# yanyan-li/PlanarSLAM

Hardware: AMD Instinct MI355X
Metric: RGB-D frames/sec (extract+match+pose-opt) @640x480; 1->8-GPU batch scaling (higher is better)
Workload: dtype u8/f64

## Files before the change

### planarslam_amd/csrc/lsd.hip

```cpp
#include "common.h"
#include "ref_arith.h"
#include "wave_ops.h"
#include "lsd_nfa.h"
#include "isort.h"

namespace planar {
namespace lsd {

constexpr double LSD_PI = 3.14159265358979323846;
constexpr double M_3_2_PI = 3 * LSD_PI / 2, M_2__PI = 2 * LSD_PI;
constexpr float NOTDEF_F = -1024.0f;
constexpr double DEG_TO_RADS = LSD_PI / 180;
constexpr double RELATIVE_ERROR_FACTOR = 100.0;
constexpr int N_BINS = 1024;
constexpr int MAX_SEGS = 2048;
constexpr int MAX_RECTS = 4096;
constexpr int RING = 512;
constexpr int USED_LDS_BITS = 32768;

struct Plan {
    int W, H, w, h;
    int taps7[7], taps5[5];
    double rho, prec, p, log_nt, density_th, log_eps;
    int min_reg_size;
// ... 1126 lines not shown
    while (hole > top && sort_comp(s.key[first + parent], vk)) {
        s.key[first + hole] = s.key[first + parent]; s.idx[first + hole] = s.idx[first + parent];
        hole = parent;
        parent = (hole - 1) / 2;
    }
    s.key[first + hole] = vk; s.idx[first + hole] = vi;
}
__device__ void heap_sort_range(const SortBuf& s, int first, int last) {
    const int len = last - first;
    if (len >= 2) {
        int parent = (len - 2) / 2;
        while (true) {
            adjust_heap(s, first, parent, len, s.key[first + parent], s.idx[first + parent]);
            if (parent == 0) break;
            parent--;
        }
    }
    int l = last;
    while (l - first > 1) {
        --l;
        const float vk = s.key[l]; const int vi = s.idx[l];
        s.key[l] = s.key[first]; s.idx[l] = s.idx[first];
        adjust_heap(s, first, 0, l - first, vk, vi);
    }
}
__device__ void std_sort_desc(const SortBuf& s, int n) {
    if (n <= 0) return;
    int stack_first[64], stack_last[64], stack_depth[64], sp = 0;
    int lg = 0; { int t = n; while (t > 1) { t >>= 1; lg++; } }
    stack_first[sp] = 0; stack_last[sp] = n; stack_depth[sp] = 2 * lg; sp++;
    while (sp > 0) {
        sp--;
        int first = stack_first[sp], last = stack_last[sp], depth = stack_depth[sp];
        while (last - first > 16) {
            if (depth == 0) { heap_sort_range(s, first, last); break; }
            --depth;
            const int mid = first + (last - first) / 2;
            const int a = first + 1, bb = mid, c = last - 1;
            if (sort_comp(s.key[a], s.key[bb])) {
                if (sort_comp(s.key[bb], s.key[c])) sort_swap(s, first, bb);
                else if (sort_comp(s.key[a], s.key[c])) sort_swap(s, first, c);
                else sort_swap(s, first, a);
            } else if (sort_comp(s.key[a], s.key[c])) sort_swap(s, first, a);
            else if (sort_comp(s.key[bb], s.key[c])) sort_swap(s, first, c);
            else sort_swap(s, first, bb);
            int lo = first + 1, hi = last;
            const float pv = s.key[first];
            while (true) {
                while (sort_comp(s.key[lo], pv)) ++lo;
                --hi;
                while (sort_comp(pv, s.key[hi])) --hi;
                if (!(lo < hi)) break;
                sort_swap(s, lo, hi);
                ++lo;
            }
            const int cut = lo;
            stack_first[sp] = cut; stack_last[sp] = last; stack_depth[sp] = depth; sp++;
            last = cut;
        }
    }
    auto linear_insert = [&](int last) {
        const float vk = s.key[last]; const int vi = s.idx[last];
        int next = last - 1;
        while (sort_comp(vk, s.key[next])) { s.key[last] = s.key[next]; s.idx[last] = s.idx[next]; last = next; --next; }
        s.key[last] = vk; s.idx[last] = vi;
    };
    auto insertion = [&](int first, int last) {
        for (int i = first + 1; i < last; ++i) {
            if (sort_comp(s.key[i], s.key[first])) {
                const float vk = s.key[i]; const int vi = s.idx[i];
                for (int j = i; j > first; --j) { s.key[j] = s.key[j - 1]; s.idx[j] = s.idx[j - 1]; }
                s.key[first] = vk; s.idx[first] = vi;
            } else linear_insert(i);
        }
    };
    if (n > 16) { insertion(0, 16); for (int i = 16; i < n; ++i) linear_insert(i); }
    else insertion(0, n);
}

__device__ inline planar_keyline make_keyline(const Seg& sg, int cols, int rows, int class_id) {
    float e[4] = {sg.x1, sg.y1, sg.x2, sg.y2};
    if (e[0] < 0) e[0] = 0;
    if (e[0] >= cols) e[0] = (float)cols - 1.0f;
    if (e[2] < 0) e[2] = 0;
    if (e[2] >= cols) e[2] = (float)cols - 1.0f;
    if (e[1] < 0) e[1] = 0;
    if (e[1] >= rows) e[1] = (float)rows - 1.0f;
    if (e[3] < 0) e[3] = 0;
    if (e[3] >= rows) e[3] = (float)rows - 1.0f;
    planar_keyline kl;
    const float octaveScale = 1.0f;
    kl.start_x = e[0] * octaveScale; kl.start_y = e[1] * octaveScale; kl.end_x = e[2] * octaveScale; kl.end_y = e[3] * octaveScale;
    kl.s_oct_x = e[0]; kl.s_oct_y = e[1]; kl.e_oct_x = e[2]; kl.e_oct_y = e[3];
    const double d0 = (double)(e[0] - e[2]), d1 = (double)(e[1] - e[3]);
    kl.line_length = (float)sqrt(d0 * d0 + d1 * d1);
    const int ax = (int)rintf(e[0]), ay = (int)rintf(e[1]), bx = (int)rintf(e[2]), by = (int)rintf(e[3]);
    kl.num_pixels = max(abs(bx - ax), abs(by - ay)) + 1;
    kl.angle = (float)atan2((double)(kl.end_y - kl.start_y), (double)(kl.end_x - kl.start_x));
    kl.class_id = class_id;
    kl.octave = 0;
    kl.size = (kl.end_x - kl.start_x) * (kl.end_y - kl.start_y);
    kl.response = kl.line_length / (float)max(cols, rows);
    kl.pt_x = (kl.end_x + kl.start_x) / 2;
    kl.pt_y = (kl.end_y + kl.start_y) / 2;
    return kl;
}

__global__ __launch_bounds__(64) void lsd_keylines(const Plan* __restrict__ plan, uint8_t* __restrict__ ws, Misc* __restrict__ miscs, int max_lines,
                                                   planar_keyline* __restrict__ out_kl, double* __restrict__ out_eq, int32_t* __restrict__ n_out, int phase) {
    constexpr int LDS_SORT = 1024;
    __shared__ float key_l[LDS_SORT];
    __shared__ int idx_l[LDS_SORT];
    const Plan& P = *plan;
    const int b = blockIdx.x, lane = threadIdx.x;
    uint8_t* F = ws + (size_t)b * P.frame_bytes;
    Misc* misc = miscs + b;
    if (phase == 1 && !(misc->imp_done && misc->imp_redo && !misc->imp_full)) return;
    const bool partial = (phase == 0 || phase == 3) && misc->imp_done && !misc->imp_full;
    const Seg* segs = (const Seg*)(F + P.off_segs);
    const int n = min(misc->n_seg, MAX_SEGS);
    const int nk = min(n, max_lines);
    planar_keyline* K = out_kl + (size_t)b * max_lines;
    planar_keyline* Kws = (planar_keyline*)(F + P.off_kl);
    auto body = [&](float* key, int* idx) {
        for (int i = lane; i < n; i += 64) { key[i] = make_keyline(segs[i], P.W, P.H, i).response; idx[i] = i; }
        __threadfence_block();
        __syncthreads();
        if (n > max_lines) {
            if (lane == 0) { SortBuf s{key, idx}; std_sort_desc(s, n); }
            __threadfence_block();
            __syncthreads();
            if (partial) {
                bool tie = false;
                for (int i = lane; i < min(n - 1, max_lines); i += 64) tie = tie || key[i] == key[i + 1];
                if ((__ballot(tie) != 0ull || phase == 3) && lane == 0) misc->imp_redo = 1;
            }
        }
        for (int i = lane; i < nk; i += 64) {
            const planar_keyline kl = make_keyline(segs[idx[i]], P.W, P.H, n > max_lines ? i : idx[i]);
            K[i] = kl; Kws[i] = kl;
            const double sp0 = kl.start_x, sp1 = kl.start_y, ep0 = kl.end_x, ep1 = kl.end_y;
            const double l0 = sp1 * 1.0 - 1.0 * ep1, l1 = 1.0 * ep0 - sp0 * 1.0, l2 = sp0 * ep1 - sp1 * ep0;
            const double nrm = sqrt(l0 * l0 + l1 * l1 + l2 * l2);
            double* E = out_eq + ((size_t)b * max_lines + i) * 3;
            E[0] = l0 / nrm; E[1] = l1 / nrm; E[2] = l2 / nrm;
        }
    };
    if (n <= LDS_SORT) body(key_l, idx_l);
    else body((float*)(F + P.off_tmp), (int*)(F + P.off_tmp) + MAX_SEGS);
    if (lane == 0) { n_out[b] = misc->status ? 0 : nk; misc->n_kl = nk; }
}

constexpr int NUM_OF_BANDS = 9, WIDTH_OF_BAND = 7, LSP_H = 63;
__constant__ int LBD_COMB[32][2] = {{0, 1}, {0, 2}, {0, 3}, {0, 4}, {0, 5}, {0, 6}, {1, 2}, {1, 3}, {1, 4}, {1, 5}, {1, 6}, {2, 3}, {2, 4}, {2, 5}, {2, 6}, {2, 7},
                                    {2, 8}, {3, 4}, {3, 5}, {3, 6}, {3, 7}, {3, 8}, {4, 5}, {4, 6}, {4, 7}, {4, 8}, {5, 6}, {5, 7}, {5, 8}, {6, 7}, {6, 8}, {7, 8}};

__global__ __launch_bounds__(64) void lbd_describe(const Plan* __restrict__ plan, uint8_t* __restrict__ ws, const Misc* __restrict__ miscs, int max_lines,
                                                   uint8_t* __restrict__ out_desc, int B) {
    __shared__ float row[LSP_H][8];
    __shared__ float des[NUM_OF_BANDS * 8];
    const Plan& P = *plan;
    int b, li;
    xcd_frame_block(max_lines, B, b, li);
    const int lane = threadIdx.x;
    uint8_t* F = ws + (size_t)b * P.frame_bytes;
    const Misc* misc = miscs + b;
    if (li >= misc->n_kl) return;
    const planar_keyline L = ((const planar_keyline*)(F + P.off_kl))[li];
    const uint8_t* S5 = F + P.off_blur5;
    const short realWidth = (short)P.W, imageWidth = (short)(P.W - 1), imageHeight = (short)(P.H - 1);
    const short lengthOfLSP = (short)L.num_pixels;
    const short halfWidth = (lengthOfLSP - 1) / 2, halfHeight = (LSP_H - 1) / 2;
    const float lineMiddlePointX = (float)(0.5 * (L.s_oct_x + L.e_oct_x));
    const float lineMiddlePointY = (float)(0.5 * (L.s_oct_y + L.e_oct_y));
    float dL[2], dO[2];
    dL[0] = (float)cos((double)L.angle); dL[1] = (float)sin((double)L.angle);
    dO[0] = -dL[1]; dO[1] = dL[0];
    if (lane < LSP_H) {
        float sCorX0 = -dL[0] * halfWidth + dL[1] * halfHeight + lineMiddlePointX;
        float sCorY0 = -dL[1] * halfWidth - dL[0] * halfHeight + lineMiddlePointY;
        for (int h = 0; h < lane; h++) { sCorX0 -= dL[1]; sCorY0 += dL[0]; }
        float sCorX = sCorX0, sCorY = sCorY0;
        float pgdLRowSum = 0, ngdLRowSum = 0, pgdORowSum = 0, ngdORowSum = 0;
        for (short wID = 0; wID < lengthOfLSP; wID++) {
            short tempCor = (short)roundf(sCorX);
            const short xCor = (tempCor < 0) ? 0 : (tempCor > imageWidth) ? imageWidth : tempCor;
            tempCor = (short)roundf(sCorY);
            const short yCor = (tempCor < 0) ? 0 : (tempCor > imageHeight) ? imageHeight : tempCor;
            const uint8_t* r0 = S5 + (size_t)reflect101(yCor - 1, P.H) * realWidth;
            const uint8_t* r1 = S5 + (size_t)yCor * realWidth;
            const uint8_t* r2 = S5 + (size_t)reflect101(yCor + 1, P.H) * realWidth;
            const int xm = reflect101(xCor - 1, P.W), xp = reflect101(xCor + 1, P.W);
            const int a0 = r0[xm], a1 = r0[xCor], a2 = r0[xp], b0 = r1[xm], b2 = r1[xp], c0 = r2[xm], c1 = r2[xCor], c2 = r2[xp];
            const short dx = (short)((a2 - a0) + 2 * (b2 - b0) + (c2 - c0)), dy = (short)((c0 - a0) + 2 * (c1 - a1) + (c2 - a2));
            const float gDL = dx * dL[0] + dy * dL[1];
            const float gDO = dx * dO[0] + dy * dO[1];
            if (gDL > 0) pgdLRowSum += gDL; else ngdLRowSum -= gDL;
            if (gDO > 0) pgdORowSum += gDO; else ngdORowSum -= gDO;
            sCorX += dL[0];
            sCorY += dL[1];
        }
        const float coef = (float)P.gaussCoefG[lane];
        pgdLRowSum = coef * pgdLRowSum; ngdLRowSum = coef * ngdLRowSum;
        pgdORowSum = coef * pgdORowSum; ngdORowSum = coef * ngdORowSum;
        row[lane][0] = pgdLRowSum; row[lane][1] = ngdLRowSum; row[lane][2] = pgdLRowSum * pgdLRowSum; row[lane][3] = ngdLRowSum * ngdLRowSum;
        row[lane][4] = pgdORowSum; row[lane][5] = ngdORowSum; row[lane][6] = pgdORowSum * pgdORowSum; row[lane][7] = ngdORowSum * ngdORowSum;
    }
    __syncthreads();
    if (lane < NUM_OF_BANDS) {
        float sum[8] = {0, 0, 0, 0, 0, 0, 0, 0};
        const int h0 = max(0, (lane - 1) * WIDTH_OF_BAND), h1 = min(LSP_H, (lane + 2) * WIDTH_OF_BAND);
        for (int hID = h0; hID < h1; hID++) {
            const int own = hID / WIDTH_OF_BAND;
            float c;
            if (own == lane) c = (float)P.gaussCoefL[hID % WIDTH_OF_BAND + WIDTH_OF_BAND];
            else if (own == lane + 1) c = (float)P.gaussCoefL[hID % WIDTH_OF_BAND + 2 * WIDTH_OF_BAND];
            else c = (float)P.gaussCoefL[hID % WIDTH_OF_BAND];
            sum[0] += c * row[hID][0]; sum[1] += c * row[hID][1]; sum[2] += c * c * row[hID][2]; sum[3] += c * c * row[hID][3];
            sum[4] += c * row[hID][4]; sum[5] += c * row[hID][5]; sum[6] += c * c * row[hID][6]; sum[7] += c * c * row[hID][7];
        }
        const float invN2 = (float)(1.0 / (WIDTH_OF_BAND * 2.0)), invN3 = (float)(1.0 / (WIDTH_OF_BAND * 3.0));
        const float invN = (lane == 0 || lane == NUM_OF_BANDS - 1) ? invN2 : invN3;
        float* d = des + lane * 8;
        float temp = sum[0] * invN;
        d[0] = temp; d[4] = sqrtf(sum[2] * invN - temp * temp);
        temp = sum[1] * invN;
        d[1] = temp; d[5] = sqrtf(sum[3] * invN - temp * temp);
        temp = sum[4] * invN;
        d[2] = temp; d[6] = sqrtf(sum[6] * invN - temp * temp);
        temp = sum[5] * invN;
        d[3] = temp; d[7] = sqrtf(sum[7] * invN - temp * temp);
    }
    __syncthreads();
    if (lane == 0) {
        float tempM = 0, tempS = 0;
        for (int i = 0; i < NUM_OF_BANDS; i++) {
            const float* d = des + 8 * i;
            tempM += d[0] * d[0]; tempM += d[1] * d[1]; tempM += d[2] * d[2]; tempM += d[3] * d[3];
            tempS += d[4] * d[4]; tempS += d[5] * d[5]; tempS += d[6] * d[6]; tempS += d[7] * d[7];
        }
        tempM = 1 / sqrtf(tempM);
        tempS = 1 / sqrtf(tempS);
        for (int i = 0; i < NUM_OF_BANDS; i++) {
            float* d = des + 8 * i;
            d[0] *= tempM; d[1] *= tempM; d[2] *= tempM; d[3] *= tempM;
            d[4] *= tempS; d[5] *= tempS; d[6] *= tempS; d[7] *= tempS;
        }
        for (int i = 0; i < NUM_OF_BANDS * 8; i++) if ((double)des[i] > 0.4) des[i] = (float)0.4;
        float temp = 0;
        for (int i = 0; i < NUM_OF_BANDS * 8; i++) temp += des[i] * des[i];
        temp = 1 / sqrtf(temp);
        for (int i = 0; i < NUM_OF_BANDS * 8; i++) des[i] = des[i] * temp;
    }
    __syncthreads();
    if (lane < 32) {
        const float *f1 = &des[8 * LBD_COMB[lane][0]], *f2 = &des[8 * LBD_COMB[lane][1]];
        uint8_t result = 0;
        for (int i = 0; i < 8; i++) if (f1[i] > f2[i]) result += (uint8_t)(128 >> i);
        out_desc[((size_t)b * max_lines + li) * 32 + lane] = result;
    }
}

#ifdef PLANAR_TEST_HOOKS
__global__ __launch_bounds__(64) void debug_sort_kernel(float* key, int* idx, int n) {
    if (threadIdx.x == 0) { SortBuf s{key, idx}; std_sort_desc(s, n); }
}
#endif

}
}

using namespace planar;

struct planar_lsd {
    planar_ctx* ctx = nullptr;
    int W = 0, H = 0, max_batch = 0;
    lsd::Plan plan{};
    int detect_smem = 0;
    DevBuf d_plan, d_cx, d_cy, d_taps, d_ws, d_misc, d_lgamma;
    DevBuf d_in, d_kl, d_desc, d_eq, d_n;
    int stage_lines = 0;
    int pre_B = 0;
    int tie_order = 0;
    int top_only = 0;
    int sort_smem_g = 0, sort_smem_l = 0, sort_rows = 0, sort_rows_long = 0;
    LaunchProfile prof{4};
};

static void host_taps_q8(int ksize, double sigma, int* taps) {
    const double scale2X = -0.5 / (sigma * sigma);
    std::vector<double> v(ksize);
    double sum = 0;
    for (int i = 0; i < ksize; i++) { const double x = i - (ksize - 1) * 0.5; v[i] = std::exp(scale2X * x * x); sum += v[i]; }
    sum = 1. / sum;
    for (int i = 0; i < ksize; i++) taps[i] = (int)std::nearbyint(v[i] * sum * 256.0);
}
static bool host_exact_coefs(double inv_scale, int srcsize, int dstsize, std::vector<lsd::Coef>& out) {
    const double scale = 1.0 / inv_scale;
    out.assign(dstsize, lsd::Coef{0, 0, 0});
    if (srcsize < 2) return false;
    for (int val = 0; val < dstsize; val++) {
        const double fval = scale * ((double)val + 0.5) - 0.5;
        const int ival = (int)std::floor(fval);
        if (ival < 0) out[val] = lsd::Coef{0, 256, 0};
        else if (ival >= srcsize - 1) out[val] = lsd::Coef{srcsize - 2, 0, 256};
        else {
            out[val].ofs = ival;
            out[val].c1 = (int)std::nearbyint((fval - (double)ival) * 256.0);
            out[val].c0 = 256 - out[val].c1;
        }
    }
    return true;
}

extern "C" {

int planar_lsd_max_segments(void) { return lsd::MAX_SEGS; }

int planar_lsd_create(planar_ctx* ctx, int width, int height, int max_batch, planar_lsd** out) {
    PLANAR_REQUIRE(ctx && out, PLANAR_EINVAL, "null argument");
    *out = nullptr;
    PLANAR_REQUIRE(width >= 32 && height >= 32 && width <= 4096 && height <= 1280, PLANAR_EINVAL, "image size out of range (32..4096 x 32..1280)");
    PLANAR_REQUIRE(max_batch >= 1, PLANAR_EINVAL, "max_batch must be >= 1");
    PLANAR_HIP_CHECK(hipSetDevice(ctx->device));
    planar_lsd* o = new (std::nothrow) planar_lsd();
    PLANAR_REQUIRE(o != nullptr, PLANAR_ENOMEM, "host allocation failed");
    o->ctx = ctx; o->W = width; o->H = height; o->max_batch = max_batch;
    lsd::Plan& P = o->plan;
    const double SCALE = 0.8, SIGMA_SCALE = 0.6, QUANT = 2.0, ANG_TH = 22.5;
    P.W = width; P.H = height;
    P.w = (int)std::nearbyint(width * SCALE); P.h = (int)std::nearbyint(height * SCALE);
    P.prec = lsd::LSD_PI * ANG_TH / 180; P.p = ANG_TH / 180; P.rho = QUANT / std::sin(P.prec);
    P.density_th = 0.7; P.log_eps = 0;
    const double sigma = SIGMA_SCALE / SCALE;
    const unsigned hk = (unsigned)(std::ceil(sigma * std::sqrt(2 * 3.0 * std::log(10.0))));
    if (1 + 2 * (int)hk != 7) { delete o; set_error("planar_lsd_create: unexpected LSD Gaussian size"); return PLANAR_EINVAL; }
    host_taps_q8(7, sigma, P.taps7);
    host_taps_q8(5, 1.0, P.taps5);
    P.log_nt = 5 * (std::log10(double(P.w)) + std::log10(double(P.h))) / 2 + std::log10(11.0);
    P.min_reg_size = (int)(size_t)(-P.log_nt / std::log10(P.p));
    {
        double u = (7 * 3 - 1) / 2, sg = (7 * 2 + 1) / 2, inv = -1 / (2 * sg * sg);
        for (int i = 0; i < 21; i++) { const double dis = i - u; P.gaussCoefL[i] = std::exp(dis * dis * inv); }
        u = (9 * 7 - 1) / 2; sg = (9 * 7) / 2; inv = -1 / (2 * sg * sg);
        for (int i = 0; i < 63; i++) { const double dis = i - u; P.gaussCoefG[i] = std::exp(dis * dis * inv); }
    }
    std::vector<lsd::Coef> cx, cy;
    if (!host_exact_coefs(SCALE, width, P.w, cx) || !host_exact_coefs(SCALE, height, P.h, cy)) {
        delete o; set_error("planar_lsd_create: image too small to resample"); return PLANAR_EINVAL;
    }
    size_t off = 0;
    auto carve = [&](size_t bytes) { size_t o2 = off; off = align_up(off + bytes, (size_t)256); return o2; };
    const size_t NPf = (size_t)width * height, NPs = (size_t)P.w * P.h;
    P.off_blur7 = carve(NPf); P.off_blur5 = carve(NPf); P.off_dx = 0; P.off_dy = 0;
// ... 273 lines not shown
```

### planarslam_amd/csrc/orb.hip

```cpp
#include <algorithm>
#include <cmath>

#include "common.h"

namespace planar {
namespace orb {

constexpr int PATCH_SIZE = 31;
constexpr int HALF_PATCH = 15;
constexpr int EDGE_THRESHOLD = 19;
constexpr int MAX_LEVELS = 16;
constexpr int CELL_W = 30;
constexpr int RADIX_BITS = 4;

struct LevelDev {
    int w, h, pitch;
    int64_t off;
    int minBX, minBY, maxBX, maxBY;
    int nCols, nRows, wCell, hCell;
    int cell_begin, ncells;
    int cand_off, cand_cap;
    int nfeat;
    int depth;
    int nIni;
// ... 490 lines not shown
        c_n = 0;
        int it = head;
        while (it >= 0) {
            __threadfence_block();
            const int sz = n_hi[it] - n_lo[it];
            if (sz == 1) { it = n_next[it]; continue; }
            nToExpand += split(it);
            it = erase(it);
        }
        if (count >= N || count == prevSize) {
            finish = true;
        } else if (count + nToExpand * 3 > N) {
            while (!finish) {
                const int prevSize2 = count;
                { int* t; t = c_size; c_size = p_size; p_size = t; t = c_seq; c_seq = p_seq; p_seq = t; t = c_slot; c_slot = p_slot; p_slot = t; }
                p_n = c_n; c_n = 0;
                __threadfence_block();
                for (int step = 0; step < p_n; step++) {
                    unsigned long long best = 0;
                    for (int i = lane; i < p_n; i += 64) {
                        const int sz = p_size[i];
                        if (sz > 0) {
                            const unsigned long long v = ((unsigned long long)sz << 40) | ((unsigned long long)p_seq[i] << 16) | (unsigned)i;
                            best = v > best ? v : best;
                        }
                    }
#pragma unroll
                    for (int o = 32; o > 0; o >>= 1) { const unsigned long long t = __shfl_xor(best, o); best = t > best ? t : best; }
                    const int idx = (int)(best & 0xffffu);
                    const int slot = p_slot[idx];
                    if (lane == 0) p_size[idx] = 0;
                    __threadfence_block();
                    split(slot);
                    erase(slot);
                    if (count >= N) break;
                }
                if (count >= N || count == prevSize2) finish = true;
            }
        }
    }

    __threadfence_block();
    int pos = 0;
    const int cw = L.wCell, ch = L.hCell, ncols = L.nCols;
    for (int it = head; it >= 0; it = n_next[it], pos++) {
        const int lo = n_lo[it], hi = n_hi[it];
        unsigned long long best = 0;
        for (int i = lo + lane; i < hi; i += 64) {
            const uint32_t key = (uint32_t)S[i];
            const unsigned x = key & 0xfffu, y = (key >> 12) & 0xfffu, sc = key >> 24;
            const unsigned cell = ((y - 3) / ch) * ncols + (x - 3) / cw;
            const unsigned long long ord = ((unsigned long long)cell << 24) | (y << 12) | x;
            const unsigned long long v = ((unsigned long long)sc << 48) | ((~ord) & 0xffffffffffffull);
            best = v > best ? v : best;
        }
#pragma unroll
        for (int o = 32; o > 0; o >>= 1) { const unsigned long long t = __shfl_xor(best, o); best = t > best ? t : best; }
        if (lane == 0) {
            const unsigned long long ord = (~best) & 0xffffffffffffull;
            out[pos] = (uint32_t)(ord & 0xffffffu) | ((uint32_t)(best >> 48) << 24);
        }
    }
    if (lane == 0) *out_count = pos;
}

struct TileDev { short level, tx, ty, pad; };

__global__ __launch_bounds__(256) void orb_blur(const PlanDev* __restrict__ plan, const TileDev* __restrict__ tiles,
                                                const uint8_t* __restrict__ pyr, uint8_t* __restrict__ blur, int n_tiles, int B) {
    __shared__ uint32_t s_pw[22][19];
    __shared__ __attribute__((aligned(8))) uint16_t s_h[22][68];
    int frame, tile;
    xcd_frame_block(n_tiles, B, frame, tile);
    const TileDev T = tiles[tile];
    const LevelDev& L = plan->lv[T.level];
    const int tid = threadIdx.x;
    const int x0 = T.tx * 64, y0 = T.ty * 16;
    const uint8_t* img = pyr + (int64_t)frame * plan->pyr_stride + L.off;
    for (int i = tid; i < 22 * 18; i += 256) {
        const int r = i / 18, wq = i - r * 18;
        int y = y0 + r - 3;
        y = y < 0 ? -y : y; y = y >= L.h ? 2 * L.h - 2 - y : y; y = max(0, min(y, L.h - 1));
        const uint8_t* row = img + (int64_t)y * L.pitch;
        const int xs = x0 - 4 + 4 * wq;
        uint32_t w;
        if (xs >= 0 && xs + 3 < L.w) w = *(const uint32_t*)(row + xs);
        else {
            w = 0;
#pragma unroll
            for (int k = 0; k < 4; k++) {
                int x = xs + k;
                x = x < 0 ? -x : x; x = x >= L.w ? 2 * L.w - 2 - x : x; x = max(0, min(x, L.w - 1));
                w |= (uint32_t)row[x] << (8 * k);
            }
        }
        s_pw[r][wq] = w;
    }
    __syncthreads();
    for (int i = tid; i < 22 * 16; i += 256) {
        const int r = i >> 4, q = i & 15;
        const uint32_t w0 = s_pw[r][q], w1 = s_pw[r][q + 1], w2 = s_pw[r][q + 2];
        uint32_t b[10];
        b[0] = (w0 >> 8) & 255u; b[1] = (w0 >> 16) & 255u; b[2] = w0 >> 24;
        b[3] = w1 & 255u; b[4] = (w1 >> 8) & 255u; b[5] = (w1 >> 16) & 255u; b[6] = w1 >> 24;
        b[7] = w2 & 255u; b[8] = (w2 >> 8) & 255u; b[9] = (w2 >> 16) & 255u;
        uint32_t o[4];
#pragma unroll
        for (int j = 0; j < 4; j++) {
            const uint32_t v = 18u * (b[j] + b[j + 6]) + 34u * (b[j + 1] + b[j + 5]) + 49u * (b[j + 2] + b[j + 4]) + 55u * b[j + 3];
            o[j] = min(v, 65535u);
        }
        *(uint2*)&s_h[r][4 * q] = make_uint2(o[0] | (o[1] << 16), o[2] | (o[3] << 16));
    }
    __syncthreads();
    {
        const int c4 = (tid & 15) * 4, r = tid >> 4;
        uint32_t acc[4] = {0, 0, 0, 0};
        const uint32_t taps[7] = {18u, 34u, 49u, 55u, 49u, 34u, 18u};
#pragma unroll
        for (int k = 0; k < 7; k++) {
            const uint2 v = *(const uint2*)&s_h[r + k][c4];
            acc[0] += taps[k] * (v.x & 0xffffu); acc[1] += taps[k] * (v.x >> 16);
            acc[2] += taps[k] * (v.y & 0xffffu); acc[3] += taps[k] * (v.y >> 16);
        }
        uint32_t packed = 0;
#pragma unroll
        for (int i = 0; i < 4; i++) packed |= min((acc[i] + 32768u) >> 16, 255u) << (8 * i);
        const int y = y0 + r, x = x0 + c4;
        if (y < L.h && x < L.pitch)
            *(uint32_t*)(blur + (int64_t)frame * plan->pyr_stride + L.off + (int64_t)y * L.pitch + x) = packed;
    }
}

__device__ __forceinline__ float fast_atan2_deg(float y, float x) {
    const float scale = (float)(180 / 3.1415926535897932384626433832795);
    const float p1 = 0.9997878412794807f * scale, p3 = -0.3258083974640975f * scale;
    const float p5 = 0.1555786518463281f * scale, p7 = -0.04432655554792128f * scale;
    const float ax = fabsf(x), ay = fabsf(y);
    float a, c, c2;
    if (ax >= ay) {
        c = __fdiv_rn(ay, __fadd_rn(ax, 2.220446049250313e-16f));
        c2 = __fmul_rn(c, c);
        a = __fmul_rn(__fadd_rn(__fmul_rn(__fadd_rn(__fmul_rn(__fadd_rn(__fmul_rn(p7, c2), p5), c2), p3), c2), p1), c);
    } else {
        c = __fdiv_rn(ax, __fadd_rn(ay, 2.220446049250313e-16f));
        c2 = __fmul_rn(c, c);
        a = __fsub_rn(90.f, __fmul_rn(__fadd_rn(__fmul_rn(__fadd_rn(__fmul_rn(__fadd_rn(__fmul_rn(p7, c2), p5), c2), p3), c2), p1), c));
    }
    if (x < 0) a = __fsub_rn(180.f, a);
    if (y < 0) a = __fsub_rn(360.f, a);
    return a;
}

__global__ __launch_bounds__(256) void orb_describe(const PlanDev* __restrict__ plan, const uint8_t* __restrict__ pyr,
                                                    const uint8_t* __restrict__ blur, const uint32_t* __restrict__ kept,
                                                    const int* __restrict__ kept_count, planar_keypoint* __restrict__ kps,
                                                    uint8_t* __restrict__ desc, int32_t* __restrict__ n_out, int per_frame, int B) {
    int frame, bx;
    xcd_frame_block(per_frame, B, frame, bx);
    const int sub = threadIdx.x & 15;
    const int kpi = bx * 16 + (threadIdx.x >> 4);
    int level = -1, first = 0, total = 0;
    for (int l = 0; l < plan->nlevels; l++) {
        const int c = kept_count[frame * MAX_LEVELS + l];
        if (level < 0 && kpi < total + c) { level = l; first = total; }
        total += c;
    }
    if (bx == 0 && threadIdx.x == 0) n_out[frame] = total;
    if (level < 0) return;
    const LevelDev& L = plan->lv[level];
    const uint32_t key = kept[(int64_t)frame * plan->kept_stride + L.kept_off + (kpi - first)];
    const int x = (int)(key & 0xfffu) + L.minBX, y = (int)((key >> 12) & 0xfffu) + L.minBY;
    const int score = (int)(key >> 24);
    const int64_t lvl_off = (int64_t)frame * plan->pyr_stride + L.off;

    const uint8_t* c = pyr + lvl_off + (int64_t)y * L.pitch + x;
    int m10 = 0, m01 = 0;
    if (sub == 0) {
        for (int u = -HALF_PATCH; u <= HALF_PATCH; ++u) m10 += u * c[u];
    } else {
        const int d = plan->umax[sub];
        int vsum = 0;
        const uint8_t* cp = c + (int64_t)sub * L.pitch;
        const uint8_t* cm = c - (int64_t)sub * L.pitch;
        for (int u = -d; u <= d; ++u) {
            const int vp = cp[u], vm = cm[u];
            vsum += vp - vm;
            m10 += u * (vp + vm);
        }
        m01 = sub * vsum;
    }
#pragma unroll
    for (int o = 8; o > 0; o >>= 1) { m10 += __shfl_xor(m10, o); m01 += __shfl_xor(m01, o); }
    const float angle = fast_atan2_deg((float)m01, (float)m10);

    const float factorPI = (float)(3.1415926535897932384626433832795 / 180.f);
    const float ang = __fmul_rn(angle, factorPI);
    const float a = (float)cos((double)ang), b = (float)sin((double)ang);
    const uint8_t* bc = blur + lvl_off + (int64_t)y * L.pitch + x;
    const int step = L.pitch;
    uint32_t bits = 0;
    const signed char* pat = c_pattern + sub * 64;
#pragma unroll
    for (int i = 0; i < 16; i++) {
        const float x0 = (float)pat[4 * i], y0 = (float)pat[4 * i + 1], x1 = (float)pat[4 * i + 2], y1 = (float)pat[4 * i + 3];
        const int r0 = __float2int_rn(__fadd_rn(__fmul_rn(x0, b), __fmul_rn(y0, a)));
        const int q0 = __float2int_rn(__fsub_rn(__fmul_rn(x0, a), __fmul_rn(y0, b)));
        const int r1 = __float2int_rn(__fadd_rn(__fmul_rn(x1, b), __fmul_rn(y1, a)));
        const int q1 = __float2int_rn(__fsub_rn(__fmul_rn(x1, a), __fmul_rn(y1, b)));
        const int t0 = bc[r0 * step + q0], t1 = bc[r1 * step + q1];
        bits |= (uint32_t)(t0 < t1) << i;
    }
    const int64_t o = (int64_t)frame * plan->kp_cap + kpi;
    *(uint16_t*)(desc + o * 32 + sub * 2) = (uint16_t)bits;
    if (sub == 0) {
        planar_keypoint kp;
        kp.x = __fmul_rn((float)x, L.scale);
        kp.y = __fmul_rn((float)y, L.scale);
        kp.size = L.patch;
        kp.angle = angle;
        kp.response = (float)score;
        kp.octave = level;
        kp.class_id = -1;
        kps[o] = kp;
    }
}

}
}

using namespace planar;
using namespace planar::orb;

struct planar_orb {
    planar_ctx* ctx = nullptr;
    planar_orb_params params{};
    int W = 0, H = 0, max_batch = 0;
    PlanDev plan{};
    std::vector<CellDev> cells;
    std::vector<TileDev> tiles;
    std::vector<float> scale, inv_scale, sigma2, inv_sigma2;
    int fast_smem = 0, node_cap = 0, oct_smem = 0;
    int last_B = 0;
    DevBuf d_plan, d_cells, d_tiles, d_tabs, d_pyr, d_blur, d_cand, d_cell_count, d_sortA, d_sortB, d_level_count,
        d_kept, d_kept_count, d_dropped;
    DevBuf d_in, d_kps, d_desc, d_nout;
    std::vector<const char*> launch_names;
    LaunchProfile prof;
    explicit planar_orb(int nlevels) : prof(nlevels + 5) {}
};

static inline int cv_round_f(float v) { return (int)nearbyintf(v); }
static inline int cv_round_d(double v) { return (int)nearbyint(v); }
static inline short sat_short(float v) { int i = cv_round_f(v); return (short)std::min(32767, std::max(-32768, i)); }

extern "C" {

int planar_orb_create(planar_ctx* ctx, const planar_orb_params* p, int W, int H, int max_batch, planar_orb** out) {
    PLANAR_REQUIRE(ctx && p && out, PLANAR_EINVAL, "null argument");
    *out = nullptr;
    PLANAR_REQUIRE(p->nlevels >= 1 && p->nlevels <= MAX_LEVELS, PLANAR_EINVAL, "nlevels must be in [1,16]");
    PLANAR_REQUIRE(p->nfeatures >= 1 && p->nfeatures <= 60000, PLANAR_EINVAL, "nfeatures out of range");
    PLANAR_REQUIRE(p->scale_factor > 1.0f, PLANAR_EINVAL, "scale_factor must be > 1");
    PLANAR_REQUIRE(p->min_th_fast >= 1 && p->ini_th_fast >= p->min_th_fast && p->ini_th_fast <= 254, PLANAR_EINVAL,
                   "FAST thresholds must satisfy 1 <= min <= ini <= 254");
    PLANAR_REQUIRE(W >= 64 && H >= 64 && W <= 4096 && H <= 4096, PLANAR_EINVAL, "image size must be within [64,4096]");
    PLANAR_REQUIRE(max_batch >= 1, PLANAR_EINVAL, "max_batch must be >= 1");
    PLANAR_HIP_CHECK(hipSetDevice(ctx->device));

    planar_orb* o = new (std::nothrow) planar_orb(p->nlevels);
    PLANAR_REQUIRE(o != nullptr, PLANAR_ENOMEM, "host allocation failed");
    o->ctx = ctx; o->params = *p; o->W = W; o->H = H; o->max_batch = max_batch;
    const int nl = p->nlevels;
    const double scaleFactor = p->scale_factor;
    o->scale.resize(nl); o->sigma2.resize(nl); o->inv_scale.resize(nl); o->inv_sigma2.resize(nl);
    o->scale[0] = 1.0f; o->sigma2[0] = 1.0f;
    for (int i = 1; i < nl; i++) { o->scale[i] = (float)(o->scale[i - 1] * scaleFactor); o->sigma2[i] = o->scale[i] * o->scale[i]; }
    for (int i = 0; i < nl; i++) { o->inv_scale[i] = 1.0f / o->scale[i]; o->inv_sigma2[i] = 1.0f / o->sigma2[i]; }
    std::vector<int> nfeat(nl);
    {
        float factor = (float)(1.0f / scaleFactor);
        float nDesired = p->nfeatures * (1 - factor) / (1 - (float)std::pow((double)factor, (double)nl));
        int sum = 0;
        for (int l = 0; l < nl - 1; l++) { nfeat[l] = cv_round_f(nDesired); sum += nfeat[l]; nDesired *= factor; }
        nfeat[nl - 1] = std::max(p->nfeatures - sum, 0);
    }
    PlanDev& P = o->plan;
    memset(&P, 0, sizeof(P));
    {
        int v, v0, vmax = (int)std::floor(HALF_PATCH * std::sqrt(2.f) / 2 + 1);
        int vmin = (int)std::ceil(HALF_PATCH * std::sqrt(2.f) / 2);
        const double hp2 = HALF_PATCH * HALF_PATCH;
        for (v = 0; v <= vmax; ++v) P.umax[v] = cv_round_d(std::sqrt(hp2 - v * v));
        for (v = HALF_PATCH, v0 = 0; v >= vmin; --v) { while (P.umax[v0] == P.umax[v0 + 1]) ++v0; P.umax[v] = v0; ++v0; }
    }
    P.nlevels = nl; P.ini_th = p->ini_th_fast; P.min_th = p->min_th_fast;

    int64_t pyr_off = 0;
    int cand_off = 0, kept_off = 0, rs_off = 0;
    int max_tile_bytes = 0, max_nfeat = 0;
    std::vector<short4> tabs;
    for (int l = 0; l < nl; l++) {
        LevelDev& L = P.lv[l];
        L.w = cv_round_f((float)W * o->inv_scale[l]);
        L.h = cv_round_f((float)H * o->inv_scale[l]);
        L.minBX = L.minBY = EDGE_THRESHOLD - 3;
        L.maxBX = L.w - EDGE_THRESHOLD + 3; L.maxBY = L.h - EDGE_THRESHOLD + 3;
        const float width = (float)(L.maxBX - L.minBX), height = (float)(L.maxBY - L.minBY);
        L.nCols = (int)(width / CELL_W); L.nRows = (int)(height / CELL_W);
        if (L.nCols < 1 || L.nRows < 1 || L.w < 2 * EDGE_THRESHOLD + 8 || L.h < 2 * EDGE_THRESHOLD + 8) {
            delete o;
            set_error("planar_orb_create: pyramid level %d (%dx%d) is too small for the 30-px FAST cell grid", l, L.w, L.h);
            return PLANAR_EINVAL;
        }
        L.wCell = (int)std::ceil(width / L.nCols); L.hCell = (int)std::ceil(height / L.nRows);
        L.pitch = align_up(L.w, 16);
        L.off = pyr_off;
        pyr_off += align_up((int64_t)L.pitch * L.h, (int64_t)256);
        L.nfeat = nfeat[l];
        max_nfeat = std::max(max_nfeat, nfeat[l]);
        L.scale = o->scale[l];
        L.patch = (float)(int)(PATCH_SIZE * o->scale[l]);
        L.nIni = (int)std::round((float)(L.maxBX - L.minBX) / (L.maxBY - L.minBY));
        if (L.nIni < 1 || L.nIni > 64) {
            delete o;
            set_error("planar_orb_create: level %d aspect ratio gives %d initial octree nodes (supported: 1..64)", l, L.nIni);
            return PLANAR_EINVAL;
        }
        L.hX = (float)(L.maxBX - L.minBX) / L.nIni;
        int ext = std::max(L.maxBX - L.minBX, L.maxBY - L.minBY), D = 1;
        while ((1 << (D - 1)) < ext) D++;
        L.depth = D;
        int ini_bits = 0; while ((1 << ini_bits) < L.nIni) ini_bits++;
        L.code_bits = align_up(2 * D + ini_bits, RADIX_BITS);
        if (L.code_bits > 32) { delete o; set_error("planar_orb_create: path code needs %d bits", L.code_bits); return PLANAR_EINVAL; }
        L.cell_begin = (int)o->cells.size();
        L.cand_off = cand_off;
        for (int i = 0; i < L.nRows; i++) {
            const float iniY = (float)(L.minBY + i * L.hCell);
            float maxY = iniY + L.hCell + 6;
            if (iniY >= L.maxBY - 3) continue;
            if (maxY > L.maxBY) maxY = (float)L.maxBY;
            for (int j = 0; j < L.nCols; j++) {
                const float iniX = (float)(L.minBX + j * L.wCell);
                float maxX = iniX + L.wCell + 6;
                if (iniX >= L.maxBX - 6) continue;
                if (maxX > L.maxBX) maxX = (float)L.maxBX;
                CellDev C;
                C.level = (short)l;
                C.x0 = (short)((int)iniX + 3); C.y0 = (short)((int)iniY + 3);
                C.ww = (short)((int)maxX - 3 - C.x0); C.wh = (short)((int)maxY - 3 - C.y0);
                if (C.ww <= 0 || C.wh <= 0) continue;
                C.slot_off = cand_off;
// ... 250 lines not shown
```

Baseline: 12870.

## Stage LBD and ORB patch pixels in LDS tiles before gradient and BRIEF sampling

The LBD describer now processes each line in 64-pixel chunks. For each chunk it computes the bounding box of all 63 rows, loads that region of the blurred image into a shared-memory tile with coalesced 32-bit loads, and computes the Sobel gradients from LDS instead of scattered global byte reads. ORB describe likewise copies each keypoint's orientation disc and BRIEF sampling box into a per-keypoint LDS tile with word loads, then takes the moments and pattern comparisons from LDS. The aim is to replace many uncoalesced byte gathers from global memory, at the cost of extra LDS use that may lower occupancy, extra sync points, and box-size limits that rely on static_assert geometry.

```diff
diff --git a/planarslam_amd/csrc/lsd.hip b/planarslam_amd/csrc/lsd.hip
--- a/planarslam_amd/csrc/lsd.hip
+++ b/planarslam_amd/csrc/lsd.hip
@@ -1302,6 +1302,9 @@
 }
 
 constexpr int NUM_OF_BANDS = 9, WIDTH_OF_BAND = 7, LSP_H = 63;
+constexpr int LBD_CH = 64, LBD_BOX = 96, LBD_PITCH_DW = 25;
+static_assert(2 * (LBD_BOX - 6) * (LBD_BOX - 6) >= (LSP_H + LBD_CH) * (LSP_H + LBD_CH), "LBD_BOX >= ceil((63 + LBD_CH) / sqrt(2)) + 4, and two to spare");
+static_assert(LBD_PITCH_DW * 4 >= LBD_BOX + 3 && (LBD_PITCH_DW & 1) == 1, "a tile row holds the box and its misalignment; odd pitch in words");
 __constant__ int LBD_COMB[32][2] = {{0, 1}, {0, 2}, {0, 3}, {0, 4}, {0, 5}, {0, 6}, {1, 2}, {1, 3}, {1, 4}, {1, 5}, {1, 6}, {2, 3}, {2, 4}, {2, 5}, {2, 6}, {2, 7},
                                     {2, 8}, {3, 4}, {3, 5}, {3, 6}, {3, 7}, {3, 8}, {4, 5}, {4, 6}, {4, 7}, {4, 8}, {5, 6}, {5, 7}, {5, 8}, {6, 7}, {6, 8}, {7, 8}};
 
@@ -1309,6 +1312,7 @@
                                                    uint8_t* __restrict__ out_desc, int B) {
     __shared__ float row[LSP_H][8];
     __shared__ float des[NUM_OF_BANDS * 8];
+    __shared__ uint32_t tile[LBD_BOX * LBD_PITCH_DW];
     const Plan& P = *plan;
     int b, li;
     xcd_frame_block(max_lines, B, b, li);
@@ -1318,7 +1322,7 @@
     if (li >= misc->n_kl) return;
     const planar_keyline L = ((const planar_keyline*)(F + P.off_kl))[li];
     const uint8_t* S5 = F + P.off_blur5;
-    const short realWidth = (short)P.W, imageWidth = (short)(P.W - 1), imageHeight = (short)(P.H - 1);
+    const short imageWidth = (short)(P.W - 1), imageHeight = (short)(P.H - 1);
     const short lengthOfLSP = (short)L.num_pixels;
     const short halfWidth = (lengthOfLSP - 1) / 2, halfHeight = (LSP_H - 1) / 2;
     const float lineMiddlePointX = (float)(0.5 * (L.s_oct_x + L.e_oct_x));
@@ -1326,30 +1330,58 @@
     float dL[2], dO[2];
     dL[0] = (float)cos((double)L.angle); dL[1] = (float)sin((double)L.angle);
     dO[0] = -dL[1]; dO[1] = dL[0];
-    if (lane < LSP_H) {
-        float sCorX0 = -dL[0] * halfWidth + dL[1] * halfHeight + lineMiddlePointX;
-        float sCorY0 = -dL[1] * halfWidth - dL[0] * halfHeight + lineMiddlePointY;
-        for (int h = 0; h < lane; h++) { sCorX0 -= dL[1]; sCorY0 += dL[0]; }
-        float sCorX = sCorX0, sCorY = sCorY0;
-        float pgdLRowSum = 0, ngdLRowSum = 0, pgdORowSum = 0, ngdORowSum = 0;
-        for (short wID = 0; wID < lengthOfLSP; wID++) {
-            short tempCor = (short)roundf(sCorX);
-            const short xCor = (tempCor < 0) ? 0 : (tempCor > imageWidth) ? imageWidth : tempCor;
-            tempCor = (short)roundf(sCorY);
-            const short yCor = (tempCor < 0) ? 0 : (tempCor > imageHeight) ? imageHeight : tempCor;
-            const uint8_t* r0 = S5 + (size_t)reflect101(yCor - 1, P.H) * realWidth;
-            const uint8_t* r1 = S5 + (size_t)yCor * realWidth;
-            const uint8_t* r2 = S5 + (size_t)reflect101(yCor + 1, P.H) * realWidth;
-            const int xm = reflect101(xCor - 1, P.W), xp = reflect101(xCor + 1, P.W);
-            const int a0 = r0[xm], a1 = r0[xCor], a2 = r0[xp], b0 = r1[xm], b2 = r1[xp], c0 = r2[xm], c1 = r2[xCor], c2 = r2[xp];
-            const short dx = (short)((a2 - a0) + 2 * (b2 - b0) + (c2 - c0)), dy = (short)((c0 - a0) + 2 * (c1 - a1) + (c2 - a2));
-            const float gDL = dx * dL[0] + dy * dL[1];
-            const float gDO = dx * dO[0] + dy * dO[1];
-            if (gDL > 0) pgdLRowSum += gDL; else ngdLRowSum -= gDL;
-            if (gDO > 0) pgdORowSum += gDO; else ngdORowSum -= gDO;
-            sCorX += dL[0];
-            sCorY += dL[1];
-        }
+    const bool has_row = lane < LSP_H;
+    float sCorX = -dL[0] * halfWidth + dL[1] * halfHeight + lineMiddlePointX;
+    float sCorY = -dL[1] * halfWidth - dL[0] * halfHeight + lineMiddlePointY;
+    for (int h = 0; h < lane; h++) { sCorX -= dL[1]; sCorY += dL[0]; }
+    float pgdLRowSum = 0, ngdLRowSum = 0, pgdORowSum = 0, ngdORowSum = 0;
+    auto clampX = [&](float v) -> short { const short t = (short)roundf(v); return (t < 0) ? (short)0 : (t > imageWidth) ? imageWidth : t; };
+    auto clampY = [&](float v) -> short { const short t = (short)roundf(v); return (t < 0) ? (short)0 : (t > imageHeight) ? imageHeight : t; };
+    const int W = P.W, H = P.H, w3 = W & 3;
+    for (int w0 = 0; w0 < lengthOfLSP; w0 += LBD_CH) {
+        const int n = min(LBD_CH, (int)lengthOfLSP - w0);
+        float eX = sCorX, eY = sCorY;
+        for (int k = 1; k < n; k++) { eX += dL[0]; eY += dL[1]; }
+        const int xs = clampX(sCorX), ys = clampY(sCorY), xe = clampX(eX), ye = clampY(eY);
+        const int xs0 = __builtin_amdgcn_readlane(xs, 0), xs1 = __builtin_amdgcn_readlane(xs, LSP_H - 1), xe0 = __builtin_amdgcn_readlane(xe, 0), xe1 = __builtin_amdgcn_readlane(xe, LSP_H - 1);
+        const int ys0 = __builtin_amdgcn_readlane(ys, 0), ys1 = __builtin_amdgcn_readlane(ys, LSP_H - 1), ye0 = __builtin_amdgcn_readlane(ye, 0), ye1 = __builtin_amdgcn_readlane(ye, LSP_H - 1);
+        const int x_lo = max(min(min(xs0, xs1), min(xe0, xe1)) - 1, 0), x_hi = min(max(max(xs0, xs1), max(xe0, xe1)) + 1, W - 1);
+        const int y_lo = max(min(min(ys0, ys1), min(ye0, ye1)) - 1, 0), y_hi = min(max(max(ys0, ys1), max(ye0, ye1)) + 1, H - 1);
+        const int bw = x_hi - x_lo + 1, bh = min(y_hi - y_lo + 1, LBD_BOX);
+        const int m0 = (int)(((uintptr_t)S5 + (size_t)y_lo * W + x_lo) & 3);
+        lds_sync();
+        const int nw = bh * LBD_PITCH_DW;
+        for (int i0 = lane; i0 < nw; i0 += 64 * 8) {
+            uint32_t v[8];
+#pragma unroll
+            for (int u = 0; u < 8; u++) {
+                const int i = min(i0 + 64 * u, nw - 1), r = i / LBD_PITCH_DW, q = i - r * LBD_PITCH_DW;
+                const int mis = (m0 + r * w3) & 3;
+                v[u] = *(const uint32_t*)(S5 + (size_t)(y_lo + r) * W + (x_lo - mis + (4 * q < mis + bw ? 4 * q : 0)));
+            }
+#pragma unroll
+            for (int u = 0; u < 8; u++) tile[min(i0 + 64 * u, nw - 1)] = v[u];
+        }
+        lds_sync();
+        if (has_row) {
+            const uint8_t* T = (const uint8_t*)tile;
+            auto row_at = [&](int y) { const int r = y - y_lo; return r * (LBD_PITCH_DW * 4) + ((m0 + r * w3) & 3) - x_lo; };
+            for (int k = 0; k < n; k++) {
+                const short xCor = clampX(sCorX), yCor = clampY(sCorY);
+                const int r0 = row_at(yCor == 0 ? 1 : yCor - 1), r1 = row_at(yCor), r2 = row_at(yCor == imageHeight ? H - 2 : yCor + 1);
+                const int xm = xCor == 0 ? 1 : xCor - 1, xp = xCor == imageWidth ? W - 2 : xCor + 1;
+                const int a0 = T[r0 + xm], a1 = T[r0 + xCor], a2 = T[r0 + xp], b0 = T[r1 + xm], b2 = T[r1 + xp], c0 = T[r2 + xm], c1 = T[r2 + xCor], c2 = T[r2 + xp];
+                const short dx = (short)((a2 - a0) + 2 * (b2 - b0) + (c2 - c0)), dy = (short)((c0 - a0) + 2 * (c1 - a1) + (c2 - a2));
+                const float gDL = dx * dL[0] + dy * dL[1];
+                const float gDO = dx * dO[0] + dy * dO[1];
+                if (gDL > 0) pgdLRowSum += gDL; else ngdLRowSum -= gDL;
+                if (gDO > 0) pgdORowSum += gDO; else ngdORowSum -= gDO;
+                sCorX += dL[0];
+                sCorY += dL[1];
+            }
+        }
+    }
+    if (has_row) {
         const float coef = (float)P.gaussCoefG[lane];
         pgdLRowSum = coef * pgdLRowSum; ngdLRowSum = coef * ngdLRowSum;
         pgdORowSum = coef * pgdORowSum; ngdORowSum = coef * ngdORowSum;
diff --git a/planarslam_amd/csrc/orb.hip b/planarslam_amd/csrc/orb.hip
--- a/planarslam_amd/csrc/orb.hip
+++ b/planarslam_amd/csrc/orb.hip
@@ -666,10 +666,29 @@
     return a;
 }
 
+constexpr signed char k_pattern_host[1024] = {
+#include "brief_pattern.inc"
+};
+constexpr int brief_reach() {
+    int m = 0;
+    for (int i = 0; i < 1024; i += 2) { const int n2 = k_pattern_host[i] * k_pattern_host[i] + k_pattern_host[i + 1] * k_pattern_host[i + 1]; m = n2 > m ? n2 : m; }
+    int r = 0;
+    while (r * r < m) r++;
+    return r;
+}
+constexpr int BRIEF_R = brief_reach();
+static_assert(BRIEF_R <= EDGE_THRESHOLD && HALF_PATCH <= EDGE_THRESHOLD, "a key point's patches must lie inside its level");
+constexpr int DISC_ROWS = 2 * HALF_PATCH + 1, DISC_DW = (3 + DISC_ROWS + 3) / 4;
+constexpr int BOX_ROWS = 2 * BRIEF_R + 1, BOX_DW = (3 + BOX_ROWS + 3) / 4;
+constexpr int KP_TILE_RAW = DISC_ROWS * DISC_DW + BOX_ROWS * BOX_DW;
+constexpr int KP_TILE_DW = KP_TILE_RAW + (8 + 32 - KP_TILE_RAW % 32) % 32;
+static_assert(KP_TILE_DW % 32 == 8 && KP_TILE_DW >= KP_TILE_RAW && 16 * KP_TILE_DW * 4 <= 64 * 1024, "key point tiles: bank offset and static LDS limit");
+
 __global__ __launch_bounds__(256) void orb_describe(const PlanDev* __restrict__ plan, const uint8_t* __restrict__ pyr,
                                                     const uint8_t* __restrict__ blur, const uint32_t* __restrict__ kept,
                                                     const int* __restrict__ kept_count, planar_keypoint* __restrict__ kps,
                                                     uint8_t* __restrict__ desc, int32_t* __restrict__ n_out, int per_frame, int B) {
+    __shared__ uint32_t s_tile[16 * KP_TILE_DW];
     int frame, bx;
     xcd_frame_block(per_frame, B, frame, bx);
     const int sub = threadIdx.x & 15;
@@ -688,15 +707,39 @@
     const int score = (int)(key >> 24);
     const int64_t lvl_off = (int64_t)frame * plan->pyr_stride + L.off;
 
-    const uint8_t* c = pyr + lvl_off + (int64_t)y * L.pitch + x;
+    uint32_t* const t_disc = s_tile + (threadIdx.x >> 4) * KP_TILE_DW;
+    uint32_t* const t_box = t_disc + DISC_ROWS * DISC_DW;
+    const int dmis = (x - HALF_PATCH) & 3, bmis = (x - BRIEF_R) & 3;
+    {
+        const uint8_t* g = pyr + lvl_off + (int64_t)(y - HALF_PATCH) * L.pitch + (x - HALF_PATCH - dmis);
+        const int nd = (dmis + DISC_ROWS + 3) >> 2;
+#pragma unroll
+        for (int j = 0; j < (DISC_ROWS * DISC_DW + 15) / 16; j++) {
+            const int i = min(sub + 16 * j, DISC_ROWS * DISC_DW - 1), r = i / DISC_DW, q = i - r * DISC_DW;
+            t_disc[i] = *(const uint32_t*)(g + (int64_t)r * L.pitch + 4 * (q < nd ? q : 0));
+        }
+    }
+    {
+        const uint8_t* g = blur + lvl_off + (int64_t)(y - BRIEF_R) * L.pitch + (x - BRIEF_R - bmis);
+        const int nd = (bmis + BOX_ROWS + 3) >> 2;
+#pragma unroll
+        for (int j = 0; j < (BOX_ROWS * BOX_DW + 15) / 16; j++) {
+            const int i = min(sub + 16 * j, BOX_ROWS * BOX_DW - 1), r = i / BOX_DW, q = i - r * BOX_DW;
+            t_box[i] = *(const uint32_t*)(g + (int64_t)r * L.pitch + 4 * (q < nd ? q : 0));
+        }
+    }
+    __builtin_amdgcn_fence(__ATOMIC_SEQ_CST, "wavefront"); __builtin_amdgcn_wave_barrier();
+
+    constexpr int DISC_STEP = DISC_DW * 4;
+    const uint8_t* c = (const uint8_t*)t_disc + HALF_PATCH * DISC_STEP + dmis + HALF_PATCH;
     int m10 = 0, m01 = 0;
     if (sub == 0) {
         for (int u = -HALF_PATCH; u <= HALF_PATCH; ++u) m10 += u * c[u];
     } else {
         const int d = plan->umax[sub];
         int vsum = 0;
-        const uint8_t* cp = c + (int64_t)sub * L.pitch;
-        const uint8_t* cm = c - (int64_t)sub * L.pitch;
+        const uint8_t* cp = c + sub * DISC_STEP;
+        const uint8_t* cm = c - sub * DISC_STEP;
         for (int u = -d; u <= d; ++u) {
             const int vp = cp[u], vm = cm[u];
             vsum += vp - vm;
@@ -711,8 +754,8 @@
     const float factorPI = (float)(3.1415926535897932384626433832795 / 180.f);
     const float ang = __fmul_rn(angle, factorPI);
     const float a = (float)cos((double)ang), b = (float)sin((double)ang);
-    const uint8_t* bc = blur + lvl_off + (int64_t)y * L.pitch + x;
-    const int step = L.pitch;
+    constexpr int step = BOX_DW * 4;
+    const uint8_t* bc = (const uint8_t*)t_box + BRIEF_R * step + bmis + BRIEF_R;
     uint32_t bits = 0;
     const signed char* pat = c_pattern + sub * 64;
 #pragma unroll
```

New measurement: 13240 (median of 6 runs). 2.8% higher.
